# aaron-randreth/modulation-mfcc

Measured on AMD Instinct MI355X. Metric: MFCC+mod-spectrum frames/sec, higher is better.
Workload: dtype f32; 1 GPU; BASELINE configs[2] per GPU: 1024 clips x 10 s x 16000 Hz, win 400 hop 160 n_fft 512, 40 mel (fmax 8000), 13 MFCC + modulation spectrum (rFFT 1024 over trajectories); frames_per_clip=1001, clips_total=1024, parallelism=clips sharded x1, hsa_ipc_mode_legacy=0, settle_calls=720, full=False, fused_tail=True

## Files before the change

modulation_mfcc_amd/csrc/mm_logmel16s.hip.inc:

```
#pragma once

struct S16Fin {
  const float* logmel;
  float* mfcc;
  float2* mod;
  const float2* tw;
  const float* dct_t;
  int n_frames, n_mels, n_mfcc, dct_kp, n_mod;
  float top_db;
  float L0;
  const float* dct_e;
};

template <int R>
__device__ __forceinline__ void s16_fin_fill_tab(const float2* tw_generic, MM_LDS mm_v2f* tab) {
  typedef f16::Geo<R> G;
  const MM_GLOBAL mm_v2f* tw = (const MM_GLOBAL mm_v2f*)tw_generic;
  for (int idx = threadIdx.x; idx < G::LPR * MM_S16_FIN_REC + 15; idx += 1024) {
    mm_v2f v;
    if (idx < G::LPR * MM_S16_FIN_REC) {
      const int q = idx / MM_S16_FIN_REC, e = idx - q * MM_S16_FIN_REC;
      if (e < 15) {
        v = tw[(q * (e + 1)) * (MM_TW_N / G::NC)];
      } else {
        const int j = e - 15, k1 = (R == 1) ? q : (q >> 1), pp = (R == 1) ? 0 : (q & 1);
        const mm_v2f w = tw[(k1 + 16 * (j + 16 * pp)) * (MM_TW_N / (2 * G::NC))];
        v = (mm_v2f){0.5f * w.y, -0.5f * w.x};
      }
    } else {
      v = tw[(idx - G::LPR * MM_S16_FIN_REC + 1) * (MM_TW_N / 32)];
    }
    tab[idx] = v;
  }
}

__device__ __forceinline__ void* mm_uniform_ptr(const void* p) {
  const unsigned long long v = (unsigned long long)p;
  const unsigned lo = __builtin_amdgcn_readfirstlane((unsigned)v), hi = __builtin_amdgcn_readfirstlane((unsigned)(v >> 32));
  return (void*)(((unsigned long long)hi << 32) | lo);
}

template <int R>
__device__ __forceinline__ void s16_fin_modspec(const S16Fin& f, int c0, int n_clips, int wave, int lane, MM_LDS float* P,
                                                const MM_LDS mm_v2f* tab) {
  typedef f16::Geo<R> G;
  const int q = lane & (G::LPR - 1), row = lane / G::LPR;
  MM_LDS mm_v2f* ex = reinterpret_cast<MM_LDS mm_v2f*>(P) + wave * G::WAVE_C;
  const MM_LDS mm_v2f* rec = tab + q * MM_S16_FIN_REC;
  const int k1 = (R == 1) ? q : (q >> 1);
  const int pp = (R == 1) ? 0 : (q & 1);
  const int n_items = (f.n_mfcc + G::ROWS - 1) / G::ROWS;
  const int T = f.n_frames;
  const int n_rows = __builtin_amdgcn_readfirstlane(f.n_mfcc * n_clips);
  const __amdgpu_buffer_rsrc_t r_in = __builtin_amdgcn_make_buffer_rsrc(
      mm_uniform_ptr(f.mfcc + (int64_t)c0 * f.n_mfcc * T), 0, n_rows * __builtin_amdgcn_readfirstlane(T) * 4, 0x00020000);
  const __amdgpu_buffer_rsrc_t r_out = __builtin_amdgcn_make_buffer_rsrc(
      mm_uniform_ptr(f.mod + (int64_t)c0 * f.n_mfcc * (G::NC + 1)), 0, n_rows * (G::NC + 1) * 8, 0x00020000);
  MM_FIN_STAMP_BEGIN
  for (int it = wave; it < n_items * n_clips; it += 16) {
    const int cl = it / n_items, g = it - cl * n_items;
    const int rr = g * G::ROWS + row;
    const bool live = rr < f.n_mfcc;
    const int r = cl * f.n_mfcc + (live ? rr : f.n_mfcc - 1);
    const int rl = r;
    const int in_off = (rl * T + 2 * q) * 4;
    float2 x[16];
#pragma unroll
    for (int n1 = 0; n1 < 16; ++n1) x[n1] = mm_buf_f32x2(r_in, in_off + 8 * G::LPR * n1);
    mm_v2f t1[15];
#pragma unroll
    for (int i = 0; i < 15; ++i) t1[i] = rec[i];
    __builtin_amdgcn_sched_barrier(0);
#pragma unroll
    for (int n1 = 0; n1 < 16; ++n1) {
      const int e = 2 * (G::LPR * n1 + q);
      x[n1].x = e < T ? x[n1].x : 0.0f;
      x[n1].y = e + 1 < T ? x[n1].y : 0.0f;
    }
    MM_FIN_STAMP(0)
    f16::dft16(x);
    MM_LDS mm_v2f* wr = ex + row * G::ROWC + q;
    wr[0] = (mm_v2f){x[f16::P16(0)].x, x[f16::P16(0)].y};
#pragma unroll
    for (int i = 1; i < 16; ++i) {
      const float2 v = f16::cmulf(x[f16::P16(i)], make_float2(t1[i - 1].x, t1[i - 1].y));
      wr[i * G::S] = (mm_v2f){v.x, v.y};
    }
    wave_lds_sync();
    if (R == 1) {
      const MM_LDS mm_v4f* rd = reinterpret_cast<const MM_LDS mm_v4f*>(ex + row * G::ROWC + q * G::S);
#pragma unroll
      for (int i = 0; i < 8; ++i) {
        const mm_v4f v = rd[i];
        x[2 * i] = make_float2(v.x, v.y);
        x[2 * i + 1] = make_float2(v.z, v.w);
      }
    } else {
      const MM_LDS mm_v2f* rd = ex + row * G::ROWC + (q >> 1) * G::S + (q & 1);
#pragma unroll
      for (int m = 0; m < 16; ++m) { const mm_v2f v = rd[2 * m]; x[m] = make_float2(v.x, v.y); }
    }
    wave_lds_sync();
    MM_FIN_STAMP(1)
    mm_v2f t2[15];
    if (R == 2) {
#pragma unroll
      for (int j = 0; j < 15; ++j) t2[j] = tab[G::LPR * MM_S16_FIN_REC + j];
      __builtin_amdgcn_sched_barrier(0);
    }
    f16::dft16(x);
    if (R == 2) {
      const float s = pp ? -1.0f : 1.0f;
#pragma unroll
      for (int j = 0; j < 16; ++j) {
        float2 v = x[f16::P16(j)];
        if (j) {
          const mm_v2f w = t2[j - 1];
          v = f16::cmulf(v, pp ? make_float2(w.x, w.y) : make_float2(1.0f, 0.0f));
        }
        x[f16::P16(j)] = make_float2(fmaf(s, v.x, f16::dpp_xor1(v.x)), fmaf(s, v.y, f16::dpp_xor1(v.y)));
      }
    }
    MM_FIN_STAMP(2)
    mm_v2f wpv[9];
#pragma unroll
    for (int j = 0; j < 9; ++j) wpv[j] = rec[15 + j];
    __builtin_amdgcn_sched_barrier(0);
    float2 b[9];
    f16::fetch_partners<R>(x, b, lane, q);
    if (live) {
      const int out_off = (r * (G::NC + 1) + k1 + 256 * pp) * 8;
#pragma unroll
      for (int j = 0; j < 9; ++j) {
        if (j == 8 && k1 != 0) break;
        const int k = k1 + 16 * (j + 16 * pp);
        float2 xa, xb;
        f16::split_pair(x[f16::P16(j)], b[j], make_float2(wpv[j].x, wpv[j].y), xa, xb);
        __builtin_amdgcn_raw_buffer_store_b64((mm_v2u){__float_as_uint(xa.x), __float_as_uint(xa.y)}, r_out,
                                              out_off + 128 * j, 0, 0);
        if (j < 8)
          __builtin_amdgcn_raw_buffer_store_b64((mm_v2u){__float_as_uint(xb.x), __float_as_uint(xb.y)}, r_out,
                                                (r * (G::NC + 1) + G::NC - k) * 8, 0, 0);
      }
    }
    MM_FIN_STAMP(3)
  }
}

__device__ __attribute__((noinline)) void s16_fix_clip(S16Fin f, int c, float thr, bool stage) {
  extern __shared__ __attribute__((aligned(16))) char fix_smem[];
  MM_LDS float* dl = (MM_LDS float*)fix_smem;
  if (stage) {
    const MM_GLOBAL float* dct_t = (const MM_GLOBAL float*)f.dct_t;
    for (int i = threadIdx.x; i < f.n_mels * f.dct_kp; i += 1024) dl[i] = dct_t[i];
    __syncthreads();
  }
  const MM_GLOBAL unsigned* ebits = f.dct_e ? (const MM_GLOBAL unsigned*)(f.dct_e + 16 * ((f.n_mfcc + 15) / 16)) : nullptr;
  const MM_GLOBAL float* dct_e = (const MM_GLOBAL float*)f.dct_e;
  const float d0 = f.dct_e ? fmaxf(thr - f.L0, 0.0f) : 0.0f;
  const int row_bytes = __builtin_amdgcn_readfirstlane(f.n_frames) * 4;
  const __amdgpu_buffer_rsrc_t r_lm = __builtin_amdgcn_make_buffer_rsrc(
      mm_uniform_ptr(f.logmel + (int64_t)c * f.n_mels * f.n_frames), 0, __builtin_amdgcn_readfirstlane(f.n_mels) * row_bytes, 0x00020000);
#pragma unroll 1
  for (int t = threadIdx.x; t < f.n_frames; t += 1024) {
    MM_GLOBAL float* o = (MM_GLOBAL float*)f.mfcc + (int64_t)c * f.n_mfcc * f.n_frames + t;
#pragma unroll 1
    for (int k0 = 0; k0 < f.n_mfcc; k0 += MM_DCT_KB) {
      float acc[MM_DCT_KB];
#pragma unroll
      for (int kk = 0; kk < MM_DCT_KB; ++kk) acc[kk] = 0.0f;
      bool touched = mm_clamp_corr(
          acc, f.n_mels, thr,
          [&](int m) { return __uint_as_float(__builtin_amdgcn_raw_buffer_load_b32(r_lm, 4 * t, __builtin_amdgcn_readfirstlane(m) * row_bytes, 0)); },
          [&](int m0) { return ebits ? ebits[m0 >> 5] : 0u; },
          [&](int m, auto fn) {
            const MM_LDS mm_v4f* d = (const MM_LDS mm_v4f*)(dl + m * f.dct_kp + k0);
#pragma unroll
            for (int q4 = 0; q4 < MM_DCT_KB / 4; ++q4) {
              const mm_v4f dv = d[q4];
              fn(4 * q4, dv.x); fn(4 * q4 + 1, dv.y); fn(4 * q4 + 2, dv.z); fn(4 * q4 + 3, dv.w);
            }
          });
      if (d0 > 0.0f) {
#pragma unroll
        for (int kk = 0; kk < MM_DCT_KB; ++kk) acc[kk] = __builtin_fmaf(dct_e[k0 + kk], d0, acc[kk]);
        touched = true;
      }
      if (touched) {
#pragma unroll
        for (int kk = 0; kk < MM_DCT_KB; ++kk)
          if (k0 + kk < f.n_mfcc) o[(int64_t)(k0 + kk) * f.n_frames] = o[(int64_t)(k0 + kk) * f.n_frames] + acc[kk];
      }
    }
  }
}

__device__ __attribute__((noinline)) void s16_add_rows(S16Fin f, int c0, int n_clips, unsigned delta_off) {
  extern __shared__ __attribute__((aligned(16))) char add_smem[];
  const float* deltas = reinterpret_cast<const float*>(add_smem + delta_off);
  const int ll = threadIdx.x & 63, wave = threadIdx.x >> 6;
  const int T = f.n_frames;
  const int n_rows = __builtin_amdgcn_readfirstlane(f.n_mfcc * n_clips);
  const MM_GLOBAL float* dct_e = (const MM_GLOBAL float*)f.dct_e;
#pragma unroll 1
  for (int r = wave; r < n_rows; r += 16) {
    const int cl = r / f.n_mfcc, k = r - cl * f.n_mfcc;
    const float delta = deltas[cl];
    if (delta == 0.0f) continue;
    const float ek = dct_e[k];
    const __amdgpu_buffer_rsrc_t r_io = __builtin_amdgcn_make_buffer_rsrc(
        mm_uniform_ptr(f.mfcc + ((int64_t)c0 * f.n_mfcc + r) * T), 0, __builtin_amdgcn_readfirstlane(T) * 4, 0x00020000);
#pragma unroll 1
    for (int e0 = 0; e0 < T; e0 += 2048) {
      float2 x[16];
#pragma unroll
      for (int n1 = 0; n1 < 16; ++n1) x[n1] = mm_buf_f32x2(r_io, (e0 + 2 * (64 * n1 + ll)) * 4);
#pragma unroll
      for (int n1 = 0; n1 < 16; ++n1) {
        const int off = (e0 + 2 * (64 * n1 + ll)) * 4;
        __builtin_amdgcn_raw_buffer_store_b32(__float_as_uint(__builtin_fmaf(ek, delta, x[n1].x)), r_io, off, 0, 0);
        __builtin_amdgcn_raw_buffer_store_b32(__float_as_uint(__builtin_fmaf(ek, delta, x[n1].y)), r_io, off + 4, 0, 0);
      }
    }
  }
}

static_assert(MM_S16_FIN2K_BYTES == (64 * MM_WPF_LT_PITCH + 16 * WpfGeo<4>::XBUF) * 4, "LDS of the 2048-point tail (mm_s16.h)");
__device__ __attribute__((noinline)) void s16_fin_modspec_2k(S16Fin f, int c0, int n_clips, unsigned delta_off) {
  typedef WpfGeo<4> G;
  extern __shared__ __attribute__((aligned(16))) char fin2k_smem[];
  float* ltab = reinterpret_cast<float*>(fin2k_smem);
  const bool has_deltas = delta_off != 0xFFFFFFFFu;
  const float* deltas = reinterpret_cast<const float*>(fin2k_smem + (has_deltas ? delta_off : 0u));
  const int ll = threadIdx.x & 63, wave = threadIdx.x >> 6;
  {
    const MM_GLOBAL float* gt = (const MM_GLOBAL float*)f.tw;
    for (int i = threadIdx.x; i < G::L * MM_WPF_LT_PITCH; i += 1024) ltab[i] = gt[i];
  }
  __syncthreads();
  const float* lt = ltab + ll * MM_WPF_LT_PITCH;
  float* xf = ltab + G::L * MM_WPF_LT_PITCH + wave * G::XBUF;
  float* zf = xf;
  const int k1 = ll / 4, pq = ll % 4;
  const int T = f.n_frames;
  const int n_rows = __builtin_amdgcn_readfirstlane(f.n_mfcc * n_clips);
  const __amdgpu_buffer_rsrc_t r_io = __builtin_amdgcn_make_buffer_rsrc(
      mm_uniform_ptr(f.mfcc + (int64_t)c0 * f.n_mfcc * T), 0, n_rows * __builtin_amdgcn_readfirstlane(T) * 4, 0x00020000);
  const __amdgpu_buffer_rsrc_t r_out = __builtin_amdgcn_make_buffer_rsrc(
      mm_uniform_ptr(f.mod + (int64_t)c0 * f.n_mfcc * (G::NC + 1)), 0, n_rows * (G::NC + 1) * 8, 0x00020000);
  const MM_GLOBAL float* dct_e = (const MM_GLOBAL float*)f.dct_e;
#pragma unroll 1
  for (int r = wave; r < n_rows; r += 16) {
    const int in_off = (r * T + 2 * ll) * 4;
    float2 x[16];
#pragma unroll
    for (int n1 = 0; n1 < 16; ++n1) x[n1] = mm_buf_f32x2(r_io, in_off + 8 * G::L * n1);
    const int cl = r / f.n_mfcc, k = r - cl * f.n_mfcc;
    const float delta = has_deltas ? deltas[cl] : 0.0f;
    if (delta != 0.0f) {
      const float ek = dct_e[k];
#pragma unroll
      for (int n1 = 0; n1 < 16; ++n1) {
        const int e = 2 * (G::L * n1 + ll);
        x[n1].x = __builtin_fmaf(ek, delta, x[n1].x);
        x[n1].y = __builtin_fmaf(ek, delta, x[n1].y);
        if (e < T) __builtin_amdgcn_raw_buffer_store_b32(__float_as_uint(x[n1].x), r_io, in_off + 8 * G::L * n1, 0, 0);
        if (e + 1 < T) __builtin_amdgcn_raw_buffer_store_b32(__float_as_uint(x[n1].y), r_io, in_off + 8 * G::L * n1 + 4, 0, 0);
      }
    }
#pragma unroll
    for (int n1 = 0; n1 < 16; ++n1) {
      const int e = 2 * (G::L * n1 + ll);
      x[n1].x = e < T ? x[n1].x : 0.0f;
      x[n1].y = e + 1 < T ? x[n1].y : 0.0f;
    }
    wpf_stages<4, false>(x, lt, xf, ll, k1, pq);
    float ar[8], br[8], ai[8], bi[8], mr, mi;
#pragma unroll
    for (int v = 0; v < 16; ++v) zf[G::zidx(k1 + 16 * (4 * pq + v / 4) + 256 * (v % 4))] = x[v].x;
    wave_lds_sync();
#pragma unroll
    for (int i = 0; i < 8; ++i) {
      const int kk = ll + G::L * i, kp = (G::NC - kk) & (G::NC - 1);
      ar[i] = zf[G::zidx(kk)];
      br[i] = zf[G::zidx(kp)];
    }
    mr = zf[G::zidx(G::NC / 2)];
    wave_lds_sync();
#pragma unroll
    for (int v = 0; v < 16; ++v) zf[G::zidx(k1 + 16 * (4 * pq + v / 4) + 256 * (v % 4))] = x[v].y;
    wave_lds_sync();
#pragma unroll
    for (int i = 0; i < 8; ++i) {
      const int kk = ll + G::L * i, kp = (G::NC - kk) & (G::NC - 1);
      ai[i] = zf[G::zidx(kk)];
      bi[i] = zf[G::zidx(kp)];
    }
    mi = zf[G::zidx(G::NC / 2)];
    wave_lds_sync();
    float2 wp[8];
    {
      const float4* s4 = reinterpret_cast<const float4*>(lt + 96);
#pragma unroll
      for (int i = 0; i < 4; ++i) { const float4 v = s4[i]; wp[2 * i] = make_float2(v.x, v.y); wp[2 * i + 1] = make_float2(v.z, v.w); }
    }
    const int out_off = r * (G::NC + 1) * 8;
#pragma unroll
    for (int i = 0; i < 8; ++i) {
      const int kk = ll + G::L * i;
      float2 xa, xb;
      f16::split_pair(make_float2(ar[i], ai[i]), make_float2(br[i], bi[i]), wp[i], xa, xb);
      __builtin_amdgcn_raw_buffer_store_b64((mm_v2u){__float_as_uint(xa.x), __float_as_uint(xa.y)}, r_out, out_off + 8 * kk, 0, 0);
      __builtin_amdgcn_raw_buffer_store_b64((mm_v2u){__float_as_uint(xb.x), __float_as_uint(xb.y)}, r_out,
                                            out_off + 8 * (G::NC - kk), 0, 0);
    }
    if (ll == 0)
      __builtin_amdgcn_raw_buffer_store_b64((mm_v2u){__float_as_uint(mr), __float_as_uint(-mi)}, r_out, out_off + 8 * (G::NC / 2), 0, 0);
  }
}

__device__ __attribute__((noinline)) void s16_finalize_all(S16Fin f, int c0, int n_clips, unsigned red_off, int clips_max) {
  extern __shared__ __attribute__((aligned(16))) char fin_smem[];
  MM_LDS char* lds = (MM_LDS char*)fin_smem;
  const int lane = threadIdx.x & 63, wave = threadIdx.x >> 6;
  const unsigned delta_off = MM_S16_DELTA_OFF(red_off, clips_max, f.n_mod);
  __syncthreads();
  bool adds = false;
  if (f.top_db >= 0.0f) {
    const MM_LDS mm_v2f* red = reinterpret_cast<const MM_LDS mm_v2f*>(lds + red_off);
    bool any = false, fixed = false;
#pragma unroll 1
    for (int cl = 0; cl < n_clips; ++cl) {
      float mx = -INFINITY, mn = INFINITY;
#pragma unroll
      for (int i = 0; i < 16; ++i) {
        const mm_v2f v = red[cl * 16 + i];
        mx = fmaxf(mx, v.x);
        mn = fminf(mn, v.y);
      }
      const float thr = mx - f.top_db;
      float delta = 0.0f;
      if (mn < thr) {
        s16_fix_clip(f, c0 + cl, thr, !fixed);
        any = true; fixed = true;
      } else if (f.dct_e && thr > f.L0) {
        delta = thr - f.L0;
        adds = true;
      }
      if (f.dct_e && threadIdx.x == 0) *reinterpret_cast<MM_LDS float*>(lds + delta_off + 4 * cl) = delta;
    }
    if (any) __syncthreads();
  }
  wg_barrier_lds();
  if (f.n_mod == 2048) {
    s16_fin_modspec_2k(f, c0, n_clips, (f.dct_e && f.top_db >= 0.0f) ? delta_off : 0xFFFFFFFFu);
    return;
  }
  if (adds) {
    s16_add_rows(f, c0, n_clips, delta_off);
    __syncthreads();
  }
  if (f.n_mod == 0) return;
  MM_LDS mm_v2f* tab = reinterpret_cast<MM_LDS mm_v2f*>(lds + MM_S16_FIN_TAB_OFF);
  if (f.n_mod == 1024) s16_fin_fill_tab<2>(f.tw, tab); else s16_fin_fill_tab<1>(f.tw, tab);
  wg_barrier_lds();
  if (f.n_mod == 1024) s16_fin_modspec<2>(f, c0, n_clips, wave, lane, (MM_LDS float*)lds, tab);
  else s16_fin_modspec<1>(f, c0, n_clips, wave, lane, (MM_LDS float*)lds, tab);
}

__device__ __forceinline__ void s16_ex_store(unsigned m0v, const float (&v)[16]) {
  unsigned keep;
  asm volatile(
      "s_mov_b32 %0, m0\n\t"
      "s_mov_b32 m0, %1\n\t"
      "s_nop 0\n\t"
      "ds_write_addtid_b32 %3 offset:%c19\n\t"
      "ds_write_addtid_b32 %4 offset:%c20\n\t"
      "ds_write_addtid_b32 %5 offset:%c21\n\t"
      "ds_write_addtid_b32 %6 offset:%c22\n\t"
      "ds_write_addtid_b32 %7 offset:%c23\n\t"
      "ds_write_addtid_b32 %8 offset:%c24\n\t"
      "ds_write_addtid_b32 %9 offset:%c25\n\t"
      "ds_write_addtid_b32 %10 offset:%c26\n\t"
      "ds_write_addtid_b32 %11 offset:%c27\n\t"
      "ds_write_addtid_b32 %12 offset:%c28\n\t"
      "ds_write_addtid_b32 %13 offset:%c29\n\t"
      "ds_write_addtid_b32 %14 offset:%c30\n\t"
      "ds_write_addtid_b32 %15 offset:%c31\n\t"
      "ds_write_addtid_b32 %16 offset:%c32\n\t"
      "ds_write_addtid_b32 %17 offset:%c33\n\t"
      "ds_write_addtid_b32 %18 offset:%c34\n\t"
      "s_mov_b32 m0, %0"
      : "=&s"(keep)
      : "s"(m0v), "i"(0),
        "v"(v[0]), "v"(v[1]), "v"(v[2]), "v"(v[3]), "v"(v[4]), "v"(v[5]), "v"(v[6]), "v"(v[7]), "v"(v[8]),
        "v"(v[9]), "v"(v[10]), "v"(v[11]), "v"(v[12]), "v"(v[13]), "v"(v[14]), "v"(v[15]),
        "i"(4 * mm_s16_xb(0)), "i"(4 * mm_s16_xb(1)), "i"(4 * mm_s16_xb(2)), "i"(4 * mm_s16_xb(3)),
        "i"(4 * mm_s16_xb(4)), "i"(4 * mm_s16_xb(5)), "i"(4 * mm_s16_xb(6)), "i"(4 * mm_s16_xb(7)),
        "i"(4 * mm_s16_xb(8)), "i"(4 * mm_s16_xb(9)), "i"(4 * mm_s16_xb(10)), "i"(4 * mm_s16_xb(11)),
        "i"(4 * mm_s16_xb(12)), "i"(4 * mm_s16_xb(13)), "i"(4 * mm_s16_xb(14)), "i"(4 * mm_s16_xb(15))
      : "memory");
}

template <int MODE, int NR, bool PRE, bool ODD, bool UNAL, bool XA>
__global__ __launch_bounds__(1024) void logmel512s_kernel(Logmel512Params p) {
  static_assert(!XA || NR >= 3, "the addtid exchange exists for NR 3 / 4 only");
  extern __shared__ __attribute__((aligned(16))) char smem[];
  float* P = reinterpret_cast<float*>(smem);
  float* S = reinterpret_cast<float*>(smem + MM_S16_S_OFF(XA));
  const int lane = threadIdx.x & 63;
  const int wave = __builtin_amdgcn_readfirstlane(threadIdx.x >> 6);
  const int q = lane & 15, row = lane >> 4;
  const float* lt = reinterpret_cast<const float*>(smem + MM_S16_LT_OFF(NR, XA)) + q * MM_W16_LT_PITCH;

  for (int i = threadIdx.x; i < 16 * MM_W16_LT_PITCH; i += 1024)
    reinterpret_cast<float*>(smem + MM_S16_LT_OFF(NR, XA))[i] = p.lane_tab[i];
  if (threadIdx.x < 64 * 3) P[(threadIdx.x / 3) * MM_S16_PITCH(XA) + 257 + threadIdx.x % 3] = 0.0f;

  for (int i = threadIdx.x; i < p.n_tab16; i += 1024)
    reinterpret_cast<float4*>(smem + MM_S16_TAB_OFF(NR, XA))[i] = p.mel_tab[i];
  const int run0 = p.wave_part[wave * 4 + 0], run1 = p.wave_part[wave * 4 + 1];
  const int m0 = p.wave_part[wave * 4 + 2];
  const bool fused = MODE == 2 || (MODE == 1 && p.out_mfcc != nullptr);
  float* Lt = reinterpret_cast<float*>(smem + p.lt_off);
  const int role = fused ? (int)((p.dct_roles >> (4 * wave)) & 15) : 15;
  const bool lt_single = fused && p.lt_b2 == 0;
  const bool halfwin = NR <= 2 && (p.dct_flags & MM_S16F_HALFWIN) != 0;
  if (fused) {
    for (int i = threadIdx.x; i < (p.lt_b2 + p.lt_rows) * 80; i += 1024) Lt[i] = 0.0f;
    for (int i = threadIdx.x; i < p.dct_kb * p.dct_nk * 64 + 16 * p.dct_kb; i += 1024)
      reinterpret_cast<float*>(smem + p.dcta_off)[i] = p.dct_a[i];
  }
  float vmin = INFINITY;
  int pb = 0, pt0 = 0;
  bool has_prev = false;
  auto dct_tile = [&](const float* Lp, int cb, int ct0) {
    int ln = lane;
    asm volatile("" : "+v"(ln));
    const int j = ln & 15, g = ln >> 4;
    const int t = ct0 + 16 * role + j;
    const float* A = reinterpret_cast<const float*>(smem + p.dcta_off) + ln;
    const float* Bp = Lp + g * 80 + 16 * role + j;
    for (int kb = 0; kb < p.dct_kb; ++kb) {
      mm_f32x4 a0 = {0.0f, 0.0f, 0.0f, 0.0f}, a1 = {0.0f, 0.0f, 0.0f, 0.0f};
      {
        const float4 e4 = *reinterpret_cast<const float4*>(A + (p.dct_kb * p.dct_nk * 64 + 16 * kb + 4 * g - ln));
        const float l0 = mm_empty_level(p.amin, p.db_offset);
        a0[0] = e4.x * l0; a0[1] = e4.y * l0; a0[2] = e4.z * l0; a0[3] = e4.w * l0;
      }
      if (p.dct_nk == 10) {
        const float* Ak = A + kb * 640;
        float av[10], bv[10];
#pragma unroll
        for (int i = 0; i < 10; ++i) {
          av[i] = Ak[i * 64];
          bv[i] = Bp[i * 320];
        }
#pragma unroll
        for (int i = 0; i < 10; i += 2) {
          a0 = __builtin_amdgcn_mfma_f32_16x16x4f32(av[i], bv[i], a0, 0, 0, 0);
          a1 = __builtin_amdgcn_mfma_f32_16x16x4f32(av[i + 1], bv[i + 1], a1, 0, 0, 0);
        }
      } else
      {
        int s0 = 0;
        for (; s0 + MM_S16F_CH <= p.dct_nk; s0 += MM_S16F_CH) {
          float av[MM_S16F_CH], bv[MM_S16F_CH];
#pragma unroll
          for (int i = 0; i < MM_S16F_CH; ++i) {
            av[i] = A[(kb * p.dct_nk + s0 + i) * 64];
            bv[i] = Bp[(s0 + i) * 320];
          }
#pragma unroll
          for (int i = 0; i < MM_S16F_CH; i += 2) {
            a0 = __builtin_amdgcn_mfma_f32_16x16x4f32(av[i], bv[i], a0, 0, 0, 0);
            a1 = __builtin_amdgcn_mfma_f32_16x16x4f32(av[i + 1], bv[i + 1], a1, 0, 0, 0);
          }
        }
        for (; s0 < p.dct_nk; s0 += 4) {
          float av[4], bv[4];
#pragma unroll
          for (int i = 0; i < 4; ++i) {
            const int s = min(s0 + i, p.dct_nk - 1);
            av[i] = s0 + i < p.dct_nk ? A[(kb * p.dct_nk + s) * 64] : 0.0f;
            bv[i] = Bp[s * 320];
          }
          a0 = __builtin_amdgcn_mfma_f32_16x16x4f32(av[0], bv[0], a0, 0, 0, 0);
          a1 = __builtin_amdgcn_mfma_f32_16x16x4f32(av[1], bv[1], a1, 0, 0, 0);
          if (s0 + 2 < p.dct_nk) {
            a0 = __builtin_amdgcn_mfma_f32_16x16x4f32(av[2], bv[2], a0, 0, 0, 0);
            a1 = __builtin_amdgcn_mfma_f32_16x16x4f32(av[3], bv[3], a1, 0, 0, 0);
          }
        }
      }
      if (t < p.n_frames) {
        float* o = p.out_mfcc + ((int64_t)cb * p.n_mfcc + 16 * kb + 4 * g) * p.n_frames + t;
#pragma unroll
        for (int r = 0; r < 4; ++r)
          if (16 * kb + 4 * g + r < p.n_mfcc) o[(int64_t)r * p.n_frames] = a0[r] + a1[r];
      }
    }
  };

  const int tpc = (int)p.tiles_per_clip;
  constexpr bool clip_mode = MODE == 2;
  const int tile_begin = clip_mode ? (int)((int64_t)blockIdx.x * p.batch / gridDim.x) * tpc
                                   : (int)((int64_t)blockIdx.x * p.n_tiles / gridDim.x);
  const int tile_end = clip_mode ? (int)((int64_t)(blockIdx.x + 1) * p.batch / gridDim.x) * tpc
                                 : (int)((int64_t)(blockIdx.x + 1) * p.n_tiles / gridDim.x);
  const int n = (int)p.n_samples;
  float vmax = -INFINITY;
  int b = tile_begin / tpc, tl = tile_begin - b * tpc;
  int nb = b, ntl = tl;

  constexpr bool addtid = XA;
  float* exw = P + 4 * wave * MM_S16_PITCH(XA) + (addtid ? mm_s16_xb(q) + 16 * row : row * 256);
  const unsigned exm0 = __builtin_amdgcn_readfirstlane((unsigned)(uintptr_t)(MM_LDS float*)(P + 4 * wave * MM_S16_PITCH(XA)));
  float* wq0 = exw + (q ^ 0);
  float* wq1 = exw + (q ^ 4);
  float* wq2 = exw + (q ^ 8);
  float* wq3 = exw + (q ^ 12);
  const int sq = addtid ? 0 : (q >> 2) & 3;
  const int rq = addtid ? 0 : q * 16;
  const float4* rq0 = reinterpret_cast<const float4*>(exw + rq + 4 * (0 ^ sq));
  const float4* rq1 = reinterpret_cast<const float4*>(exw + rq + 4 * (1 ^ sq));
  const float4* rq2 = reinterpret_cast<const float4*>(exw + rq + 4 * (2 ^ sq));
  const float4* rq3 = reinterpret_cast<const float4*>(exw + rq + 4 * (3 ^ sq));
  const float* sxf = S + (4 * wave + row) * p.hop + 2 * q;
  const float2* sx = reinterpret_cast<const float2*>(sxf);
  constexpr bool hop_odd = ODD;

  float4 sreg[NR];
  float sprev[PRE ? NR : 1];
  auto stage_interior = [&](int ttl) -> bool {
    const int base = ttl * 64 * p.hop - 256;
    return base >= 0 && base + NR * 4096 <= n;
  };
  auto stage_load = [&](int bb, int ttl) {
    const float* a = p.audio + (int64_t)bb * p.stride;
    const int first = ttl * 64 * p.hop - 256 + 4 * (int)threadIdx.x;
    int off[NR];
    if (stage_interior(ttl)) {
#pragma unroll
      for (int j = 0; j < NR; ++j) off[j] = first + 4096 * j;
    } else {
#pragma unroll
      for (int j = 0; j < NR; ++j) off[j] = min(max(first + 4096 * j, 0), n - 4);
    }
    __builtin_amdgcn_sched_barrier(0);
#pragma unroll
    for (int j = 0; j < NR; ++j) {
      if (UNAL) {
        const MmFloat4U t = *reinterpret_cast<const MmFloat4U*>(a + off[j]);
        sreg[j] = make_float4(t.x, t.y, t.z, t.w);
      } else {
        sreg[j] = *reinterpret_cast<const float4*>(a + off[j]);
      }
    }
    if (PRE) {
#pragma unroll
      for (int j = 0; j < NR; ++j) sprev[j] = a[min(max(first + 4096 * j - 1, 0), n - 1)];
    }
    __builtin_amdgcn_sched_barrier(0);
  };
  auto stage_store = [&](int ttl) {
    const int first = ttl * 64 * p.hop - 256 + 4 * (int)threadIdx.x;
    if (!PRE && stage_interior(ttl)) {
#pragma unroll
      for (int j = 0; j < NR; ++j) reinterpret_cast<float4*>(S)[threadIdx.x + 1024 * j] = sreg[j];
      return;
    }
#pragma unroll
    for (int j = 0; j < NR; ++j) {
      const int s0 = first + 4096 * j;
      const bool ok = s0 >= 0 && s0 < n;
      float4 v = sreg[j];
      if (UNAL) {
        const int k = s0 - (n - 4);
        if (k > 0) {
          const float4 l = v;
          v.x = k == 1 ? l.y : (k == 2 ? l.z : l.w);
          v.y = k == 1 ? l.z : l.w;
          v.z = l.w;
        }
      }
      if (PRE) {
        const float pv = s0 > 0 ? sprev[j] : 0.0f;
        const float4 r = v;
        v.x = r.x - __fmul_rn(p.preemph, pv); v.y = r.y - __fmul_rn(p.preemph, r.x);
        v.z = r.z - __fmul_rn(p.preemph, r.y); v.w = r.w - __fmul_rn(p.preemph, r.z);
      }
      if (UNAL) {
        v.x = ok ? v.x : 0.0f; v.y = (ok && s0 + 1 < n) ? v.y : 0.0f;
        v.z = (ok && s0 + 2 < n) ? v.z : 0.0f; v.w = (ok && s0 + 3 < n) ? v.w : 0.0f;
      } else {
        v.x = ok ? v.x : 0.0f; v.y = ok ? v.y : 0.0f; v.z = ok ? v.z : 0.0f; v.w = ok ? v.w : 0.0f;
      }
      reinterpret_cast<float4*>(S)[threadIdx.x + 1024 * j] = v;
    }
  };
  if (tile_begin < tile_end) {
    stage_load(b, tl);
    stage_store(tl);
  }
  __syncthreads();
  float2 twr[MM_S16_TW_REG > 0 ? MM_S16_TW_REG : 1];
#if MM_S16_WP_REG
  float2 wp[8];
#endif
  {
#if MM_S16_WP_REG
    const float4* s4 = reinterpret_cast<const float4*>(lt + 64);
#pragma unroll
    for (int i = 0; i < 4; ++i) {
      const float4 t = s4[i];
      wp[2 * i] = make_float2(t.x, t.y);
      wp[2 * i + 1] = make_float2(t.z, t.w);
    }
#endif
    const float4* t4 = reinterpret_cast<const float4*>(lt + 32);
#pragma unroll
    for (int i = 0; i < MM_S16_TW_REG / 2; ++i) {
      const float4 t = t4[i];
      twr[2 * i] = make_float2(t.x, t.y);
      twr[2 * i + 1] = make_float2(t.z, t.w);
    }
  }

  MM_STAMP_BEGIN(16)
  for (int tile = tile_begin; tile < tile_end; ++tile) {
    const int t0 = tl * 64;
    MM_STAMP_AT(9)
    if (++ntl == tpc) { ntl = 0; ++nb; }
    const bool more = tile + 1 < tile_end;
    stage_load(more ? nb : b, more ? ntl : tl);
    MM_STAMP_AT(11)
    if (t0 + 4 * wave < (int)p.n_frames) {
    float2 x[16];
    if (halfwin) {
      if (hop_odd) {
#pragma unroll
        for (int n1 = 4; n1 < 12; ++n1) x[n1] = make_float2(sxf[32 * n1], sxf[32 * n1 + 1]);
      } else {
#pragma unroll
        for (int n1 = 4; n1 < 12; ++n1) x[n1] = sx[16 * n1];
      }
      const float4* w4 = reinterpret_cast<const float4*>(lt) + 2;
#pragma unroll
      for (int i = 0; i < 4; ++i) {
        const float4 t = w4[i];
        x[4 + 2 * i].x *= t.x; x[4 + 2 * i].y *= t.y;
        x[5 + 2 * i].x *= t.z; x[5 + 2 * i].y *= t.w;
      }
      MM_STAMP_AT(0)
      f16::dft16_mid8(x);
    } else {
    if (hop_odd) {
#pragma unroll
      for (int n1 = 0; n1 < 16; ++n1) x[n1] = make_float2(sxf[32 * n1], sxf[32 * n1 + 1]);
    } else {
#pragma unroll
      for (int n1 = 0; n1 < 16; ++n1) x[n1] = sx[16 * n1];
    }
    {
      float2 w[16];
      w16_read16(w, lt);
#pragma unroll
      for (int n1 = 0; n1 < 16; ++n1) { x[n1].x *= w[n1].x; x[n1].y *= w[n1].y; }
    }
    MM_STAMP_AT(0)
    f16::dft16(x);
    }
    MM_STAMP_AT(1)
    {
      float2 w[16];
      const float4* t4 = reinterpret_cast<const float4*>(lt + 32);
#pragma unroll
      for (int i = MM_S16_TW_REG / 2; i < 8; ++i) {
        const float4 t = t4[i];
        w[2 * i] = make_float2(t.x, t.y);
        w[2 * i + 1] = make_float2(t.z, t.w);
      }
#pragma unroll
      for (int k1 = 1; k1 < 16; ++k1)
        x[f16::P16(k1)] = f16::cmulf(x[f16::P16(k1)], (k1 - 1 < MM_S16_TW_REG) ? twr[(k1 - 1) % (MM_S16_TW_REG > 0 ? MM_S16_TW_REG : 1)] : w[k1 - 1]);
    }
    MM_STAMP_AT(2)
    {
#define MM_S16_WR(k1, val)                                                                         \
  (((k1) >> 2) == 0 ? wq0 : ((k1) >> 2) == 1 ? wq1 : ((k1) >> 2) == 2 ? wq2 : wq3)[(k1) * 16] = (val)
      {
        float re[16];
#pragma unroll
        for (int k1 = 0; k1 < 16; ++k1) re[k1] = x[f16::P16(k1)].x;
        if constexpr (addtid) {
          s16_ex_store(exm0, re);
        } else {
#pragma unroll
          for (int k1 = 0; k1 < 16; ++k1) MM_S16_WR(k1, re[k1]);
        }
      }
      wave_lds_sync();
      {
        const float4 v0 = *rq0, v1 = *rq1, v2 = *rq2, v3 = *rq3;
        x[0].x = v0.x; x[1].x = v0.y; x[2].x = v0.z; x[3].x = v0.w;
        x[4].x = v1.x; x[5].x = v1.y; x[6].x = v1.z; x[7].x = v1.w;
        x[8].x = v2.x; x[9].x = v2.y; x[10].x = v2.z; x[11].x = v2.w;
        x[12].x = v3.x; x[13].x = v3.y; x[14].x = v3.z; x[15].x = v3.w;
      }
      wave_lds_sync();
      float im[16];
#pragma unroll
      for (int k1 = 0; k1 < 16; ++k1) im[k1] = x[f16::P16(k1)].y;
      if constexpr (addtid) {
        s16_ex_store(exm0, im);
      } else {
#pragma unroll
        for (int k1 = 0; k1 < 16; ++k1) MM_S16_WR(k1, im[k1]);
      }
      wave_lds_sync();
      {
        const float4 v0 = *rq0, v1 = *rq1, v2 = *rq2, v3 = *rq3;
        x[0].y = v0.x; x[1].y = v0.y; x[2].y = v0.z; x[3].y = v0.w;
        x[4].y = v1.x; x[5].y = v1.y; x[6].y = v1.z; x[7].y = v1.w;
        x[8].y = v2.x; x[9].y = v2.y; x[10].y = v2.z; x[11].y = v2.w;
        x[12].y = v3.x; x[13].y = v3.y; x[14].y = v3.z; x[15].y = v3.w;
      }
      wave_lds_sync();
#undef MM_S16_WR
    }
    MM_STAMP_AT(10)
    f16::dft16(x);
    MM_STAMP_AT(3)
    {
      float2 pb[9];
      f16::fetch_partners<1>(x, pb, lane, q);
#if !MM_S16_WP_REG
      float2 wp[8];
      {
        const float4* s4 = reinterpret_cast<const float4*>(lt + 64);
#pragma unroll
        for (int i = 0; i < 4; ++i) {
          const float4 t = s4[i];
          wp[2 * i] = make_float2(t.x, t.y);
          wp[2 * i + 1] = make_float2(t.z, t.w);
        }
      }
#endif
      float* pr = P + (4 * wave + row) * MM_S16_PITCH(XA);
      float pw[17];
#pragma unroll
      for (int j = 0; j < 8; ++j) {
        float2 xa, xb;
        f16::split_pair(x[f16::P16(j)], pb[j], wp[j], xa, xb);
        pw[2 * j] = fmaf(xa.x, xa.x, xa.y * xa.y);
        pw[2 * j + 1] = fmaf(xb.x, xb.x, xb.y * xb.y);
      }
      {
        const float2 zm = x[f16::P16(8)];
        pw[16] = fmaf(zm.x, zm.x, zm.y * zm.y);
      }
#pragma unroll
      for (int j = 0; j < 8; ++j) {
        pr[q + 16 * j] = pw[2 * j];
        pr[256 - q - 16 * j] = pw[2 * j + 1];
      }
      if (q == 0) {
        pr[128] = pw[16];
        pr[257] = 0.0f; pr[258] = 0.0f; pr[259] = 0.0f;
      }
    }
    }
    MM_STAMP_AT(4)
    if (!lt_single) {
      wg_barrier_lds();
      MM_STAMP_AT(6)
      stage_store(more ? ntl : tl);
    }
    if (MODE != 0 && role < 4 && has_prev) dct_tile(Lt + (((tile & 1) ^ 1) * p.lt_b2) * 80, pb, pt0);
    if (lt_single) {
      wg_barrier_lds();
      stage_store(more ? ntl : tl);
    }
    MM_STAMP_AT(5)
    if (MODE == 0) {
      for (int r = wave; r < 64; r += 16) {
        if (t0 + r < p.n_frames) {
          float* o = p.out_power + (((int64_t)b * p.n_frames) + t0 + r) * 257;
          const float* src = P + r * MM_S16_PITCH(XA);
          for (int k = lane; k < 257; k += 64) o[k] = src[k];
        }
      }
    } else {
      const bool valid = (t0 + lane) < p.n_frames;
      float* o = p.out_logmel + ((int64_t)b * p.n_mels + m0) * p.n_frames + t0 + lane;
      const float* pl = P + lane * MM_S16_PITCH(XA);
      const float4* hdr = reinterpret_cast<const float4*>(smem + MM_S16_TAB_OFF(NR, XA));
      const float4* grp = hdr + p.n_runs;
      float carry = 0.0f;
      if (run0 < run1) {
        float4 h = hdr[run0];
        for (int r = run0; r < run1; ++r) {
          const int k4e = __builtin_amdgcn_readfirstlane(__float_as_int(h.x));
          const int k4 = k4e & 0xFFFF;
          const bool empty_d = (k4e >> 16) & 1;
          const int ng = __builtin_amdgcn_readfirstlane(__float_as_int(h.y));
          const int go = __builtin_amdgcn_readfirstlane(__float_as_int(h.z));
          const int dd = __builtin_amdgcn_readfirstlane(__float_as_int(h.w));
          if (r + 1 < run1) h = hdr[r + 1];
          const float4* pp = reinterpret_cast<const float4*>(pl + k4);
          const MM_LDS mm_v4f* gw = (const MM_LDS mm_v4f*)(grp + 2 * go);
          asm volatile("" : "+v"(gw));
          float sa = 0.0f, sb = 0.0f;
          MM_STAMP_AT(12)
#pragma unroll 2
          for (int g = 0; g < ng; ++g) {
            const float4 pv = pp[g];
            const mm_v4f wa = gw[2 * g], wb = gw[2 * g + 1];
            sa = fmaf(wa.x, pv.x, sa); sb = fmaf(wa.y, pv.x, sb);
            sa = fmaf(wa.z, pv.y, sa); sb = fmaf(wa.w, pv.y, sb);
            sa = fmaf(wb.x, pv.z, sa); sb = fmaf(wb.y, pv.z, sb);
            sa = fmaf(wb.z, pv.w, sa); sb = fmaf(wb.w, pv.w, sb);
          }
          MM_STAMP_AT(13)
          float dbm = __builtin_nanf("");
          if (dd >= m0) {
            if (!empty_d) {
              const float v = carry + sa;
              const float db = 3.0102999566398120f * __builtin_amdgcn_logf(mm_max_raw_s(v, p.amin)) - p.db_offset;
              if (valid && p.out_logmel) *o = db;
              dbm = valid ? db : dbm;
              if (fused) Lt[((tile & 1) * p.lt_b2 + dd) * 80 + lane] = db;
            }
            o += p.n_frames;
          }
          mm_max_acc(vmax, dbm);
          mm_min_acc(vmin, dbm);
          carry = sb;
          MM_STAMP_AT(14)
        }
      }
      const bool clip_done = (tile + 1 == tile_end) || (ntl == 0);
      if (clip_done) {
        vmax = wave_max(vmax);
        if (p.key_nmin || clip_mode) vmin = wave_min(vmin);
        if (clip_mode) {
          if (lane == 0)
            reinterpret_cast<float2*>(smem + p.red_off)[(b - tile_begin / tpc) * 16 + wave] = make_float2(vmax, vmin);
        } else if (lane == 0 && vmax > -INFINITY) {
          atomicMax(p.clip_key + b, float_key(vmax));
          if (p.key_nmin) atomicMax(p.key_nmin + b, float_key(-vmin));
        }
        vmax = -INFINITY; vmin = INFINITY;
      }
    }
    MM_STAMP_AT(7)
    wg_barrier_lds();
    MM_STAMP_AT(8)
    pb = b; pt0 = t0; has_prev = true;
    b = nb; tl = ntl;
  }
  if (role < 4 && has_prev) dct_tile(Lt + (((tile_end - 1) & 1) * p.lt_b2) * 80, pb, pt0);
  if (clip_mode && has_prev) {
    S16Fin f;
    f.logmel = p.out_logmel; f.mfcc = p.out_mfcc; f.mod = p.out_mod; f.tw = p.tw; f.dct_t = p.dct_t;
    f.n_frames = (int)p.n_frames; f.n_mels = p.n_mels; f.n_mfcc = p.n_mfcc; f.dct_kp = p.dct_kp; f.n_mod = p.n_mod;
    f.top_db = p.top_db;
    f.dct_e = (p.dct_flags & MM_S16F_SKIP) ? p.dct_a + p.dct_kb * p.dct_nk * 64 : nullptr;
    f.L0 = mm_empty_level(p.amin, p.db_offset);
    s16_finalize_all(f, tile_begin / tpc, (tile_end - tile_begin) / tpc, p.red_off,
                     (int)((p.batch + gridDim.x - 1) / gridDim.x));
  }
  MM_STAMP_END(16)
}

template <int MODE, int NR, bool XA>
static void launch_s16_mn(bool pre, bool odd, bool unal, dim3 grid, size_t lds, hipStream_t st, const Logmel512Params& q) {
#define MM_S16_GO(PP, OO, UU) hipLaunchKernelGGL((logmel512s_kernel<MODE, NR, PP, OO, UU, XA>), grid, dim3(1024), lds, st, q)
  if (NR < 3) {
    switch ((odd ? 2 : 0) | (unal ? 1 : 0)) {
      case 0: MM_S16_GO(false, false, false); break;
      case 1: MM_S16_GO(false, false, true); break;
      case 2: MM_S16_GO(false, true, false); break;
      default: MM_S16_GO(false, true, true); break;
    }
    return;
  }
  constexpr int NRP = NR < 3 ? 3 : NR;
#define MM_S16_GOP(OO, UU) hipLaunchKernelGGL((logmel512s_kernel<MODE, NRP, true, OO, UU, XA>), grid, dim3(1024), lds, st, q)
  switch ((pre ? 4 : 0) | (odd ? 2 : 0) | (unal ? 1 : 0)) {
    case 0: MM_S16_GO(false, false, false); break;
    case 1: MM_S16_GO(false, false, true); break;
    case 2: MM_S16_GO(false, true, false); break;
    case 3: MM_S16_GO(false, true, true); break;
    case 4: MM_S16_GOP(false, false); break;
    case 5: MM_S16_GOP(false, true); break;
    case 6: MM_S16_GOP(true, false); break;
    default: MM_S16_GOP(true, true); break;
  }
#undef MM_S16_GOP
#undef MM_S16_GO
}

template <int NR, bool XA>
static void launch_s16_n(int mode, bool pre, bool odd, bool unal, dim3 grid, size_t lds, hipStream_t st, const Logmel512Params& q) {
  if (mode == 0) launch_s16_mn<0, NR, XA>(pre, odd, unal, grid, lds, st, q);
  else if (mode == 1) launch_s16_mn<1, NR, XA>(pre, odd, unal, grid, lds, st, q);
  else launch_s16_mn<2, NR, XA>(pre, odd, unal, grid, lds, st, q);
}

void launch_s16(int mode, int nr, bool xa, bool pre, bool odd, bool unal, dim3 grid, size_t lds, hipStream_t st,
                const Logmel512Params& q) {
  if (mode == 1 && q.out_mod != nullptr) mode = 2;
  switch (nr) {
    case 1: launch_s16_n<1, false>(mode, pre, odd, unal, grid, lds, st, q); break;
    case 2: launch_s16_n<2, false>(mode, pre, odd, unal, grid, lds, st, q); break;
    case 3:
      if (xa) launch_s16_n<3, true>(mode, pre, odd, unal, grid, lds, st, q);
      else launch_s16_n<3, false>(mode, pre, odd, unal, grid, lds, st, q);
      break;
    default:
      if (xa) launch_s16_n<4, true>(mode, pre, odd, unal, grid, lds, st, q);
      else launch_s16_n<4, false>(mode, pre, odd, unal, grid, lds, st, q);
      break;
  }
}

template <int MODE, int NR, bool XA>
static bool set_s16_attr_mn(int bytes) {
  constexpr int NRP = NR < 3 ? 3 : NR;
  const void* fn[8] = {(const void*)logmel512s_kernel<MODE, NR, false, false, false, XA>, (const void*)logmel512s_kernel<MODE, NR, false, false, true, XA>,
                       (const void*)logmel512s_kernel<MODE, NR, false, true, false, XA>, (const void*)logmel512s_kernel<MODE, NR, false, true, true, XA>,
                       (const void*)logmel512s_kernel<MODE, NRP, true, false, false, XA>, (const void*)logmel512s_kernel<MODE, NRP, true, false, true, XA>,
                       (const void*)logmel512s_kernel<MODE, NRP, true, true, false, XA>, (const void*)logmel512s_kernel<MODE, NRP, true, true, true, XA>};
  for (int i = 0; i < 8; ++i)
    if (hipFuncSetAttribute(fn[i], hipFuncAttributeMaxDynamicSharedMemorySize, bytes) != hipSuccess) return false;
  return true;
}

bool set_s16_attr(int bytes) {
  return set_s16_attr_mn<0, 1, false>(bytes) && set_s16_attr_mn<1, 1, false>(bytes) && set_s16_attr_mn<2, 1, false>(bytes) &&
         set_s16_attr_mn<0, 2, false>(bytes) && set_s16_attr_mn<1, 2, false>(bytes) && set_s16_attr_mn<2, 2, false>(bytes) &&
         set_s16_attr_mn<0, 3, false>(bytes) && set_s16_attr_mn<1, 3, false>(bytes) && set_s16_attr_mn<2, 3, false>(bytes) &&
         set_s16_attr_mn<0, 4, false>(bytes) && set_s16_attr_mn<1, 4, false>(bytes) && set_s16_attr_mn<2, 4, false>(bytes) &&
         set_s16_attr_mn<0, 3, true>(bytes) && set_s16_attr_mn<1, 3, true>(bytes) && set_s16_attr_mn<2, 3, true>(bytes) &&
         set_s16_attr_mn<0, 4, true>(bytes) && set_s16_attr_mn<1, 4, true>(bytes) && set_s16_attr_mn<2, 4, true>(bytes);
}
```

Baseline: 2.490 billion frames/s.

## Skip logmel stores in clip mode; recompute only clips needing top_db clamp

In fused clip mode the kernel no longer writes log-mel values to global memory on the first pass. After all tiles are processed it checks each clip's max/min, and for clips where top_db clamping would be needed it loops back and recomputes that clip, this time storing log-mel values. This cuts global write traffic in the common case, at the cost of a full recompute for any clip that needs clamping. It also assumes the finalize step can work from the fused DCT outputs when the stored log-mel is absent.

Result: no change. 2.481 billion frames/s (median of 2 runs) (-0.4%).

```diff
diff --git a/modulation_mfcc_amd/csrc/mm_logmel16s.hip.inc b/modulation_mfcc_amd/csrc/mm_logmel16s.hip.inc
--- a/modulation_mfcc_amd/csrc/mm_logmel16s.hip.inc
+++ b/modulation_mfcc_amd/csrc/mm_logmel16s.hip.inc
@@ -504,14 +504,16 @@
 
   const int tpc = (int)p.tiles_per_clip;
   constexpr bool clip_mode = MODE == 2;
-  const int tile_begin = clip_mode ? (int)((int64_t)blockIdx.x * p.batch / gridDim.x) * tpc
-                                   : (int)((int64_t)blockIdx.x * p.n_tiles / gridDim.x);
-  const int tile_end = clip_mode ? (int)((int64_t)(blockIdx.x + 1) * p.batch / gridDim.x) * tpc
-                                 : (int)((int64_t)(blockIdx.x + 1) * p.n_tiles / gridDim.x);
+  int tile_begin = clip_mode ? (int)((int64_t)blockIdx.x * p.batch / gridDim.x) * tpc
+                             : (int)((int64_t)blockIdx.x * p.n_tiles / gridDim.x);
+  int tile_end = clip_mode ? (int)((int64_t)(blockIdx.x + 1) * p.batch / gridDim.x) * tpc
+                           : (int)((int64_t)(blockIdx.x + 1) * p.n_tiles / gridDim.x);
   const int n = (int)p.n_samples;
   float vmax = -INFINITY;
   int b = tile_begin / tpc, tl = tile_begin - b * tpc;
   int nb = b, ntl = tl;
+  const int c0 = b, n_clips = clip_mode ? (tile_end - tile_begin) / tpc : 0;
+  bool replay = false;
 
   constexpr bool addtid = XA;
   float* exw = P + 4 * wave * MM_S16_PITCH(XA) + (addtid ? mm_s16_xb(q) + 16 * row : row * 256);
@@ -599,6 +601,7 @@
       reinterpret_cast<float4*>(S)[threadIdx.x + 1024 * j] = v;
     }
   };
+  for (;;) {
   if (tile_begin < tile_end) {
     stage_load(b, tl);
     stage_store(tl);
@@ -777,7 +780,7 @@
       MM_STAMP_AT(6)
       stage_store(more ? ntl : tl);
     }
-    if (MODE != 0 && role < 4 && has_prev) dct_tile(Lt + (((tile & 1) ^ 1) * p.lt_b2) * 80, pb, pt0);
+    if (MODE != 0 && role < 4 && has_prev && !replay) dct_tile(Lt + (((tile & 1) ^ 1) * p.lt_b2) * 80, pb, pt0);
     if (lt_single) {
       wg_barrier_lds();
       stage_store(more ? ntl : tl);
@@ -828,11 +831,15 @@
             if (!empty_d) {
               const float v = carry + sa;
               const float db = 3.0102999566398120f * __builtin_amdgcn_logf(mm_max_raw_s(v, p.amin)) - p.db_offset;
-              if (valid && p.out_logmel) *o = db;
+              if (clip_mode) {
+                if (replay && valid) p.out_logmel[((int64_t)b * p.n_mels + dd) * p.n_frames + t0 + lane] = db;
+              } else if (valid && p.out_logmel) {
+                *o = db;
+              }
               dbm = valid ? db : dbm;
               if (fused) Lt[((tile & 1) * p.lt_b2 + dd) * 80 + lane] = db;
             }
-            o += p.n_frames;
+            if (!clip_mode) o += p.n_frames;
           }
           mm_max_acc(vmax, dbm);
           mm_min_acc(vmin, dbm);
@@ -845,8 +852,8 @@
         vmax = wave_max(vmax);
         if (p.key_nmin || clip_mode) vmin = wave_min(vmin);
         if (clip_mode) {
-          if (lane == 0)
-            reinterpret_cast<float2*>(smem + p.red_off)[(b - tile_begin / tpc) * 16 + wave] = make_float2(vmax, vmin);
+          if (lane == 0 && !replay)
+            reinterpret_cast<float2*>(smem + p.red_off)[(b - c0) * 16 + wave] = make_float2(vmax, vmin);
         } else if (lane == 0 && vmax > -INFINITY) {
           atomicMax(p.clip_key + b, float_key(vmax));
           if (p.key_nmin) atomicMax(p.key_nmin + b, float_key(-vmin));
@@ -860,15 +867,36 @@
     pb = b; pt0 = t0; has_prev = true;
     b = nb; tl = ntl;
   }
-  if (role < 4 && has_prev) dct_tile(Lt + (((tile_end - 1) & 1) * p.lt_b2) * 80, pb, pt0);
-  if (clip_mode && has_prev) {
+  if (role < 4 && has_prev && !replay) dct_tile(Lt + (((tile_end - 1) & 1) * p.lt_b2) * 80, pb, pt0);
+  if (!clip_mode || !has_prev || !(p.top_db >= 0.0f)) break;
+  unsigned long long clamps = 0;
+  {
+    float mx = -INFINITY, mn = INFINITY;
+    if (lane < n_clips) {
+      const float2* red = reinterpret_cast<const float2*>(smem + p.red_off) + lane * 16;
+#pragma unroll
+      for (int i = 0; i < 16; ++i) {
+        const float2 v = red[i];
+        mx = fmaxf(mx, v.x);
+        mn = fminf(mn, v.y);
+      }
+    }
+    clamps = __builtin_amdgcn_ballot_w64(lane < n_clips && (!replay || lane > pb - c0) && mn < mx - p.top_db);
+  }
+  if (clamps == 0) break;
+  replay = true;
+  b = nb = c0 + __builtin_ctzll(clamps); tl = ntl = 0;
+  tile_begin = 0; tile_end = tpc;
+  has_prev = false;
+  }
+  if (clip_mode && n_clips > 0) {
     S16Fin f;
     f.logmel = p.out_logmel; f.mfcc = p.out_mfcc; f.mod = p.out_mod; f.tw = p.tw; f.dct_t = p.dct_t;
     f.n_frames = (int)p.n_frames; f.n_mels = p.n_mels; f.n_mfcc = p.n_mfcc; f.dct_kp = p.dct_kp; f.n_mod = p.n_mod;
     f.top_db = p.top_db;
     f.dct_e = (p.dct_flags & MM_S16F_SKIP) ? p.dct_a + p.dct_kb * p.dct_nk * 64 : nullptr;
     f.L0 = mm_empty_level(p.amin, p.db_offset);
-    s16_finalize_all(f, tile_begin / tpc, (tile_end - tile_begin) / tpc, p.red_off,
+    s16_finalize_all(f, c0, n_clips, p.red_off,
                      (int)((p.batch + gridDim.x - 1) / gridDim.x));
   }
   MM_STAMP_END(16)
```
